# hjsuh94/irs_mpc

Hardware: AMD Instinct MI355X
Metric: rollouts*timesteps/s (randomized-smoothing pass) + iLQR-iters/s (higher is better)
Workload: dtype f32; 1 GPU; planar_hand quasi-dynamic contact, zero-order-B smoothing, step QP solved exactly (dual active-set method) -- the metric's config; T=50, N_per_gpu=10000, N_total=10000, mode=ZERO_ORDER_B, contact_solver=exact, samples=supplied, resident in HBM (f32), parallelism=samples sharded over 1 GPU(s), 1 all-reduce of (T,P) f64 per step

## Files before the change

irs_mpc_amd/csrc/reduce.hpp:

```cpp
#pragma once
#include <hip/hip_runtime.h>

constexpr int irs_reduce_pad(int P) {
    if (P > 32) return (P + 63) / 64 * 64;
    int q = 1;
    while (q < P) q <<= 1;
    return q;
}

template <int LEN, int STAGE>
struct WaveReduce {
    static constexpr bool HALVE = (LEN % 2 == 0);
    static constexpr int NEXT = HALVE ? LEN / 2 : LEN;
    static constexpr int FINAL_LEN = WaveReduce<NEXT, STAGE + 1>::FINAL_LEN;

    __device__ __forceinline__ static void run(float* v, int lane) {
        constexpr int mask = 32 >> STAGE;
        if constexpr (HALVE) {
            const bool upper = (lane & mask) != 0;
#pragma unroll
            for (int i = 0; i < LEN / 2; ++i) {
                float keep = upper ? v[i + LEN / 2] : v[i];
                float send = upper ? v[i] : v[i + LEN / 2];
                v[i] = keep + __shfl_xor(send, mask, 64);
            }
        } else {
#pragma unroll
            for (int i = 0; i < LEN; ++i) v[i] += __shfl_xor(v[i], mask, 64);
        }
        WaveReduce<NEXT, STAGE + 1>::run(v, lane);
    }
    __device__ __forceinline__ static int base(int lane) {
        constexpr int mask = 32 >> STAGE;
        int rest = WaveReduce<NEXT, STAGE + 1>::base(lane);
        if constexpr (HALVE) {
            return (rest < 0) ? -1 : rest + ((lane & mask) ? LEN / 2 : 0);
        } else {
            return (lane & mask) ? -1 : rest;
        }
    }
};
template <int LEN>
struct WaveReduce<LEN, 6> {
    static constexpr int FINAL_LEN = LEN;
    __device__ __forceinline__ static void run(float*, int) {}
    __device__ __forceinline__ static int base(int) { return 0; }
};

template <int P, int NW>
__device__ __forceinline__ void block_reduce_lds(float* acc, float* red) {
    constexpr int PP = irs_reduce_pad(P);
    using WR = WaveReduce<PP, 0>;
    const int tid = threadIdx.x;
    const int lane = tid & 63, wave = tid >> 6;
    WR::run(acc, lane);
    const int b = WR::base(lane);
    if (b >= 0) {
#pragma unroll
        for (int i = 0; i < WR::FINAL_LEN; ++i) red[wave * PP + b + i] = acc[i];
    }
}
```

irs_mpc_amd/csrc/smooth_common.hpp:

```cpp
#pragma once
#include <type_traits>
#include <cstdlib>
#include "irs_common.hpp"
#include "philox.hpp"
#include "reduce.hpp"

struct SmoothArgs {
    ModelParams p;
    const double* x_trj;
    const double* u_trj;
    const float* dx;
    const float* du;
    float std[32];
    unsigned long long seed;
    unsigned long long sample_offset;
    unsigned int iter;
    int T, N, chunk, nblk, block;
    int diag;
    int* counters;
    float* partial;
    double* fnom;
    int chunk0;
    int wg0_rr;
    double* sums;
// ... 258 lines not shown
        if (lane == 0) {
#pragma unroll
            for (int k = 0; k < n; ++k) L.fd[k] = f[k] - (double)(float)x[k];
        }
        wave_sync();
        for (int q = lane; q < NZ * n; q += 64) {
            double hq = S[TR::NG + q];
            if constexpr (TR::SUMZ) hq -= S[TR::NH + q / n] * L.fd[q % n];
            L.H[q / n][q % n] = hq;
        }
        wave_sync();
        if (lane < NZ) {
            double g = L.G[lane][lane];
            L.sc[lane] = g > 0.0 ? 1.0 / sqrt(g) : 0.0;
            if (!(g > 0.0)) L.bad = lane + 1;
        }
        wave_sync();
        for (int q = lane; q < NZ * NZ; q += 64) L.G[q / NZ][q % NZ] *= L.sc[q / NZ] * L.sc[q % NZ];
        for (int q = lane; q < NZ * n; q += 64) L.H[q / n][q % n] *= L.sc[q / n];
        wave_sync();
        static_assert(NZ <= 32 && n <= 32, "lane split of the scaling step");
        for (int j = 0; j < NZ; ++j) {
            double djj = L.G[j][j];
            if (!(djj > 1e-14)) {
                if (lane == 0 && L.bad == 0) L.bad = j + 1;
                djj = 1.0;
            }
            const double il = fast_rsqrt(djj);
            wave_sync();
            if (lane == j) L.G[j][j] = il;
            if (lane > j && lane < NZ) L.G[lane][j] *= il;
            if (lane >= 32 && lane < 32 + n) L.H[j][lane - 32] *= il;
            wave_sync();
            for (int q = lane; q < NZ * NZ; q += 64) {
                int r = q / NZ, c = q % NZ;
                if (c > j && r >= c) L.G[r][c] -= L.G[r][j] * L.G[c][j];
            }
            for (int q = lane; q < NZ * n; q += 64) {
                int r = q / n, k = q % n;
                if (r > j) L.H[r][k] -= L.G[r][j] * L.H[j][k];
            }
            wave_sync();
        }
        for (int i = NZ - 1; i >= 0; --i) {
            const double il = L.G[i][i];
            wave_sync();
            if (lane < n) L.H[i][lane] *= il;
            wave_sync();
            for (int q = lane; q < i * n; q += 64) {
                int r = q / n, k = q % n;
                L.H[r][k] -= L.G[i][r] * L.H[i][k];
            }
        }
        wave_sync();
        for (int q = lane; q < NZ * n; q += 64) L.AB[q % n][Z0 + q / n] = L.H[q / n][q % n] * L.sc[q / n];
        }
    }
    wave_sync();
    if constexpr ((MODE == IRS_SMOOTH_ZERO_ORDER_B && !Model::HAS_JACOBIAN) || TR::FIRST_B) {
        for (int q = lane; q < m * m; q += 64) L.AB[Model::u_into_x(q / m)][n + q % m] = (q / m == q % m) ? 1.0 : 0.0;
        wave_sync();
    }
    for (int q = lane; q < n * n; q += 64) At[(size_t)t * n * n + q] = L.AB[q / n][q % n];
    for (int q = lane; q < n * m; q += 64) Bt[(size_t)t * n * m + q] = L.AB[q / m][n + q % m];
    if (lane < n) {
        double c = f[0];
#pragma unroll
        for (int i = 0; i < n; ++i) c = (i == lane) ? f[i] : c;
#pragma unroll
        for (int i = 0; i < n; ++i) c -= L.AB[lane][i] * x[i];
#pragma unroll
        for (int j = 0; j < m; ++j) c -= L.AB[lane][n + j] * u[j];
        ct[(size_t)t * n + lane] = c;
    }
    {
        bool nonfinite = false;
        for (int q = lane; q < TR::P; q += 64) {
            const unsigned long long bits = (unsigned long long)__double_as_longlong(S[q]);
            nonfinite = nonfinite || ((bits & 0x7ff0000000000000ull) == 0x7ff0000000000000ull);
        }
        if (__any(nonfinite) && lane == 0) L.bad = TR::P + 1;
    }
    wave_sync();
    if (lane == 0) info[t] = L.bad;
}

struct SmoothRow {
    const ModelParams& p;
    const double* x_trj;
    const double* u_trj;
    const float* dx;
    const float* du;
    float std[32];
    unsigned long long seed, sample_offset;
    unsigned int iter;
    int T, N, chunk, nblk, block, diag;
    int* counters;
    float* partial;
    double* fnom;
    int chunk0, wg0_rr;
    double* sums;
    double* At;
    double* Bt;
    double* ct;
    int* info;
    double n_total;
    int t;
};

template <class Model, int MODE>
__device__ __forceinline__ SmoothRow smooth_batch_row(const SmoothArgs& a, const SmoothBatch& bat, int row) {
    using TR = SmoothTraits<Model, MODE>;
    constexpr int n = TR::n, m = TR::m;
    const int b = row / a.T;
    const long long wsb = b * bat.ws_stride;
    const size_t rows = (size_t)b * a.T;
    SmoothRow r{.p = a.p,
                .x_trj = a.x_trj + b * bat.x_stride,
                .u_trj = a.u_trj + b * bat.u_stride,
                .dx = nullptr, .du = nullptr,
                .std = {},
                .seed = bat.seed[b], .sample_offset = 0ull, .iter = a.iter,
                .T = a.T, .N = a.N, .chunk = a.chunk, .nblk = a.nblk, .block = a.block, .diag = a.diag,
                .counters = reinterpret_cast<int*>(reinterpret_cast<char*>(a.counters) + wsb),
                .partial = reinterpret_cast<float*>(reinterpret_cast<char*>(a.partial) + wsb),
                .fnom = reinterpret_cast<double*>(reinterpret_cast<char*>(a.fnom) + wsb),
                .chunk0 = a.chunk0, .wg0_rr = a.wg0_rr,
                .sums = a.sums + rows * TR::P, .At = a.At + rows * (n * n), .Bt = a.Bt + rows * (n * m),
                .ct = a.ct + rows * n, .info = a.info + rows,
                .n_total = a.n_total, .t = row - b * a.T};
#pragma unroll
    for (int j = 0; j < m; ++j)
        r.std[n + j] = __int_as_float(__builtin_amdgcn_readfirstlane(__float_as_int((float)bat.std_u[(size_t)b * m + j])));
    return r;
}

template <class Model, int MODE>
__device__ __forceinline__ const SmoothArgs& smooth_row(const SmoothArgs& a, const SmoothSolo&, int) { return a; }
template <class Model, int MODE>
__device__ __forceinline__ SmoothRow smooth_row(const SmoothArgs& a, const SmoothBatch& bat, int row) {
    return smooth_batch_row<Model, MODE>(a, bat, row);
}
__device__ __forceinline__ int smooth_row_t(const SmoothArgs&, int row) { return row; }
__device__ __forceinline__ int smooth_row_t(const SmoothRow& r, int) { return r.t; }

template <class Model, class = void>
struct contact_rows_of { static constexpr int value = 0; };
template <class Model>
struct contact_rows_of<Model, std::void_t<decltype(Model::NC)>> { static constexpr int value = Model::NC; };
template <class Model>
constexpr int contact_rows() { return contact_rows_of<Model>::value; }


template <class Model, int MODE, bool FUSE, int BLOCK, bool FNOM_ONLY = false, class Args = SmoothArgs>
__device__ __forceinline__ void smooth_finish(const Args& a, float* red, double* red64, double* tot,
                                              FinalizeLds<Model, MODE>& fin, int& s_ticket, int t, int blk, int tid,
                                              const double* fnom_t) {
    using TR = SmoothTraits<Model, MODE>;
    constexpr int n = TR::n, P = TR::P;
    constexpr int NW = BLOCK / 64;
    constexpr int P4 = (P + 3) / 4 * 4;
    (void)n;
    __syncthreads();

    const int nblk = a.nblk;
    if (nblk == 1) {
        for (int q = tid; q < P; q += BLOCK) {
            float s = red[q];
#pragma unroll
            for (int w = 1; w < NW; ++w) s += red[w * TR::PP + q];
            tot[q] = (double)s;
        }
    } else if constexpr (BLOCK <= 512 || FNOM_ONLY) {
        for (int q = tid; q < P; q += BLOCK) {
            float s = red[q];
#pragma unroll
            for (int w = 1; w < NW; ++w) s += red[w * TR::PP + q];
            red[q] = s;
        }
        __syncthreads();
        {
            typedef unsigned int u32x4 __attribute__((ext_vector_type(4)));
            const unsigned bytes = (unsigned)((size_t)a.T * nblk * P4 * sizeof(float));
            __amdgpu_buffer_rsrc_t rsrc = __builtin_amdgcn_make_buffer_rsrc(a.partial, 0, bytes, 0x00020000);
            const unsigned row = (unsigned)(((size_t)t * nblk + blk) * P4 * sizeof(float));
            for (int q4 = tid; q4 < P4 / 4; q4 += BLOCK) {
                u32x4 v;
                v.x = __float_as_uint(red[4 * q4]);
                v.y = __float_as_uint(red[4 * q4 + 1]);
                v.z = __float_as_uint(red[4 * q4 + 2]);
                v.w = __float_as_uint(red[4 * q4 + 3]);
                __builtin_amdgcn_raw_buffer_store_b128(v, rsrc, row + 16u * q4, 0, 16 );
            }
        }
        asm volatile("s_waitcnt vmcnt(0)" ::: "memory");
        __syncthreads();
        if (tid == 0)
            s_ticket = __hip_atomic_fetch_add(a.counters + t, 1, __ATOMIC_RELAXED, __HIP_MEMORY_SCOPE_AGENT);
        __syncthreads();
        if (s_ticket != nblk - 1) return;
        if (tid == 0) {
            __hip_atomic_store(a.counters + t, 0, __ATOMIC_RELAXED, __HIP_MEMORY_SCOPE_AGENT);
            __builtin_amdgcn_fence(__ATOMIC_ACQUIRE, "agent");
        }
        asm volatile("s_waitcnt vmcnt(0)" ::: "memory");
        __syncthreads();
        const float* src = a.partial + (size_t)t * nblk * P4;
        if constexpr (P >= kBlock) {
            for (int q = tid; q < P; q += BLOCK) {
                double s = 0.0;
#pragma unroll 8
                for (int b = 0; b < nblk; ++b) s += (double)src[(size_t)b * P4 + q];
                tot[q] = s;
            }
        } else {
            const int g = tid / P, q = tid % P;
            if (g < TR::NGRP) {
                double s = 0.0;
#pragma unroll 4
                for (int b = g; b < nblk; b += TR::NGRP) s += (double)src[(size_t)b * P4 + q];
                red64[g * P + q] = s;
            }
            __syncthreads();
            if (tid < P) {
                double s = red64[tid];
                for (int gg = 1; gg < TR::NGRP; ++gg) s += red64[gg * P + tid];
                tot[tid] = s;
            }
        }
    }
    __syncthreads();
    for (int q = tid; q < P; q += BLOCK) a.sums[(size_t)t * P + q] = tot[q];
    if constexpr (FUSE) {
        if (tid < 64 && a.diag != 1)
            finalize_timestep<Model, MODE, FNOM_ONLY>(a.p, a.x_trj, a.u_trj, tot, a.n_total, t, tid, fin, a.At, a.Bt,
                                           a.ct, a.info,
                                           fnom_t);
    }
}

}
```

irs_mpc_amd/csrc/smooth_ug.hip:

```cpp
#include "smooth_common.hpp"

namespace {

#ifndef IRS_UG_SWEEPS
#define IRS_UG_SWEEPS 6
#endif
#ifndef IRS_UG_PDAS
#define IRS_UG_PDAS 4
#endif
#ifndef IRS_UG_BLOCK
#define IRS_UG_BLOCK 512
#endif
constexpr int kUgBlock = IRS_UG_BLOCK;
constexpr int kUgSweeps = IRS_UG_SWEEPS;
constexpr int kUgPdas = IRS_UG_PDAS;
#ifndef IRS_UG_STEP_COLUMNS
#define IRS_UG_STEP_COLUMNS 1
#endif
constexpr bool kUgStepColumns = IRS_UG_STEP_COLUMNS != 0;
constexpr int kUgTabH = 8, kUgTabTau = 40, kUgTabSet = 48, kUgTabX = 52;
constexpr int kUgTabStride = 116;
#ifndef IRS_UG_NOM_ROUNDS
#define IRS_UG_NOM_ROUNDS 2
#endif
constexpr int kUgNomRounds = IRS_UG_NOM_ROUNDS;
constexpr int kUgRing = 128;

template <class Model>
struct alignas(16) UgLds {
    static constexpr int NC = Model::NC, n = Model::NX, m = Model::NU;
    float tab[1 << NC][kUgTabStride];
    float W[NC][NC];
    float invw[NC];
    float Wd[NC];
    float r0[NC];
    float phi[NC];
    float C[m][NC];
    float JD[n][NC];
    float Jc[NC][n];
    float Dinv[n];
    float Db0[n];
    float DK[m];
    float q[n];
};

__device__ __forceinline__ float ug_uniform(float v) {
    return __int_as_float(__builtin_amdgcn_readfirstlane(__float_as_int(v)));
}

template <int NC>
struct UgUni {
    float W[NC * (NC + 1) / 2];
    float invw[NC];
    float r0[NC];
    __device__ __forceinline__ float w(int i, int j) const {
        return i <= j ? W[i * NC - i * (i - 1) / 2 + (j - i)] : W[j * NC - j * (j - 1) / 2 + (i - j)];
    }
};

template <class Model>
__device__ __forceinline__ unsigned ug_lookup_affine(const UgLds<Model>& S, unsigned a, const float* du, float tol,
                                                     float* v, float* tau) {
    constexpr int NC = Model::NC, m = Model::NU;
    static_assert(NC == 8 && m == 4, "table entries are 8 rows by 4 commands");
    const float4* e = reinterpret_cast<const float4*>(&S.tab[a][0]);
    float4 g4[kUgTabSet / 4];
#pragma unroll
    for (int c = 0; c < kUgTabSet / 4; ++c) g4[c] = e[c];
    const unsigned ap = __float_as_uint(S.tab[a][kUgTabSet]);
    tau[0] = g4[kUgTabTau / 4].x; tau[1] = g4[kUgTabTau / 4].y; tau[2] = g4[kUgTabTau / 4].z; tau[3] = g4[kUgTabTau / 4].w;
    tau[4] = g4[kUgTabTau / 4 + 1].x; tau[5] = g4[kUgTabTau / 4 + 1].y; tau[6] = g4[kUgTabTau / 4 + 1].z; tau[7] = g4[kUgTabTau / 4 + 1].w;
    v[0] = fmaf(tau[0], tol, g4[0].x); v[1] = fmaf(tau[1], tol, g4[0].y);
    v[2] = fmaf(tau[2], tol, g4[0].z); v[3] = fmaf(tau[3], tol, g4[0].w);
    v[4] = fmaf(tau[4], tol, g4[1].x); v[5] = fmaf(tau[5], tol, g4[1].y);
    v[6] = fmaf(tau[6], tol, g4[1].z); v[7] = fmaf(tau[7], tol, g4[1].w);
#pragma unroll
    for (int j = 0; j < m; ++j) {
        const float4 lo = g4[kUgTabH / 4 + 2 * j], hi = g4[kUgTabH / 4 + 2 * j + 1];
        v[0] = fmaf(lo.x, du[j], v[0]); v[1] = fmaf(lo.y, du[j], v[1]);
        v[2] = fmaf(lo.z, du[j], v[2]); v[3] = fmaf(lo.w, du[j], v[3]);
        v[4] = fmaf(hi.x, du[j], v[4]); v[5] = fmaf(hi.y, du[j], v[5]);
        v[6] = fmaf(hi.z, du[j], v[6]); v[7] = fmaf(hi.w, du[j], v[7]);
    }
    return ap;
}

template <class Model, bool UCOL>
__device__ __forceinline__ void ug_step_direction(const UgLds<Model>& S, unsigned a, int p, float* u, float* tau) {
    constexpr int NC = Model::NC;
    const float* e = &S.tab[a][0];
    const float4 t0 = *reinterpret_cast<const float4*>(e + kUgTabTau), t1 = *reinterpret_cast<const float4*>(e + kUgTabTau + 4);
    if constexpr (UCOL) {
        const float4 lo = *reinterpret_cast<const float4*>(e + kUgTabX + NC * p);
        const float4 hi = *reinterpret_cast<const float4*>(e + kUgTabX + NC * p + 4);
        u[0] = lo.x; u[1] = lo.y; u[2] = lo.z; u[3] = lo.w;
        u[4] = hi.x; u[5] = hi.y; u[6] = hi.z; u[7] = hi.w;
    } else {
        const float4 wlo = *reinterpret_cast<const float4*>(&S.W[p][0]);
        const float4 whi = *reinterpret_cast<const float4*>(&S.W[p][4]);
        const float4* x4 = reinterpret_cast<const float4*>(e + kUgTabX);
        float4 g4[2 * NC];
#pragma unroll
        for (int c = 0; c < 2 * NC; ++c) g4[c] = x4[c];
        const float wp[NC] = {wlo.x, wlo.y, wlo.z, wlo.w, whi.x, whi.y, whi.z, whi.w};
#pragma unroll
        for (int i = 0; i < NC; ++i) u[i] = 0.f;
#pragma unroll
        for (int c = 0; c < NC; ++c) {
            const float4 lo = g4[2 * c], hi = g4[2 * c + 1];
            u[0] = fmaf(lo.x, wp[c], u[0]); u[1] = fmaf(lo.y, wp[c], u[1]);
            u[2] = fmaf(lo.z, wp[c], u[2]); u[3] = fmaf(lo.w, wp[c], u[3]);
            u[4] = fmaf(hi.x, wp[c], u[4]); u[5] = fmaf(hi.y, wp[c], u[5]);
            u[6] = fmaf(hi.z, wp[c], u[6]); u[7] = fmaf(hi.w, wp[c], u[7]);
        }
    }
    tau[0] = t0.x; tau[1] = t0.y; tau[2] = t0.z; tau[3] = t0.w;
    tau[4] = t1.x; tau[5] = t1.y; tau[6] = t1.z; tau[7] = t1.w;
}

template <class Model>
__device__ __forceinline__ float ug_rhs(const UgUni<Model::NC>& U, const UgLds<Model>& S, const float* du, float* r) {
    constexpr int NC = Model::NC, m = Model::NU;
#pragma unroll
    for (int c = 0; c < NC; ++c) r[c] = U.r0[c];
#pragma unroll
    for (int j = 0; j < m; ++j) {
        const float4 lo = *reinterpret_cast<const float4*>(&S.C[j][0]);
        const float4 hi = *reinterpret_cast<const float4*>(&S.C[j][4]);
        r[0] = fmaf(lo.x, du[j], r[0]); r[1] = fmaf(lo.y, du[j], r[1]);
        r[2] = fmaf(lo.z, du[j], r[2]); r[3] = fmaf(lo.w, du[j], r[3]);
        r[4] = fmaf(hi.x, du[j], r[4]); r[5] = fmaf(hi.y, du[j], r[5]);
        r[6] = fmaf(hi.z, du[j], r[6]); r[7] = fmaf(hi.w, du[j], r[7]);
    }
    float scale = 1e-30f;
#pragma unroll
    for (int c = 0; c < NC; ++c) scale = fmaxf(scale, fabsf(r[c]));
    return 1e-6f * scale;
}

template <class Model>
__device__ __forceinline__ bool ug_try(const UgUni<Model::NC>& U, const UgLds<Model>& S, const float* r, const float* du,
                                       float tolv, float* lam, unsigned& a_out, int diag = 0) {
    constexpr int NC = Model::NC;
    float g[NC];
#pragma unroll
    for (int i = 0; i < NC; ++i) { lam[i] = 0.f; g[i] = r[i]; }
#pragma unroll 2
    for (int sw = 0; sw < ((diag & 64) ? 0 : kUgSweeps); ++sw) {
#pragma unroll
        for (int i = 0; i < NC; ++i) {
            const float nw = fmaxf(fmaf(-g[i], U.invw[i], lam[i]), 0.f);
            const float dl = nw - lam[i];
            lam[i] = nw;
#pragma unroll
            for (int j = 0; j < NC; ++j) g[j] = fmaf(U.w(j, i), dl, g[j]);
        }
    }
    unsigned a = 0u;
#pragma unroll
    for (int i = 0; i < NC; ++i) a |= (lam[i] > 0.f) ? (1u << i) : 0u;
    bool done = (diag & 32) != 0;
    for (int it = 0; it < kUgPdas; ++it) {
        float v[NC], tau[NC];
        const unsigned ap = ug_lookup_affine<Model>(S, a, du, tolv, v, tau);
        unsigned bad = 0u;
#pragma unroll
        for (int i = NC - 1; i >= 0; --i) bad = __builtin_amdgcn_alignbit(bad, __float_as_uint(v[i]), 31);
        if (!done) {
            if (bad == 0u) {
#pragma unroll
                for (int i = 0; i < NC; ++i) lam[i] = fmaf(-tau[i], v[i], v[i]);
                done = true;
            }
            a = ap ^ bad;
        }
        if (__all(done)) break;
    }
    a_out = a;
    return done;
}

template <class Model, bool UCOL>
__device__ __forceinline__ void ug_full(const UgLds<Model>& S, const float* r, const float* du, float tolv, unsigned a,
                                        float* lam, int cap = 4 * Model::NC) {
    constexpr int NC = Model::NC;
    constexpr float kBig = 3.0e38f, piv_rel = 1e-5f;
    float g[NC];
    bool valid = false;
    for (int round = 0; round < 3; ++round) {
        if (__all(valid)) break;
        float v[NC], tau[NC];
        const unsigned ap = ug_lookup_affine<Model>(S, a, du, 0.f, v, tau);
        if (!valid) {
            unsigned negb = 0u;
#pragma unroll
            for (int i = 0; i < NC; ++i) {
                const bool in = tau[i] == 0.f;
                negb |= (in && !(v[i] > 0.f)) ? (1u << i) : 0u;
                lam[i] = in ? v[i] : 0.f;
                g[i] = in ? 0.f : v[i];
            }
            valid = negb == 0u;
            a = ap & ~negb;
        }
    }
    if (!valid) {
        a = 0u;
#pragma unroll
        for (int i = 0; i < NC; ++i) { lam[i] = 0.f; g[i] = r[i]; }
    }
    int p = -1;
    bool done = false;
    for (int it = 0; it < cap; ++it) {
        if (!done && p < 0) {
            float vmin = kBig;
            int c = 0;
#pragma unroll
            for (int i = 0; i < NC; ++i) {
                const float vv = ((a >> i) & 1u) ? kBig : g[i];
                if (vv < vmin) { vmin = vv; c = i; }
            }
            if (vmin >= -tolv) done = true;
            else p = c;
        }
        if (__all(done)) break;
        const int pp = (done || p < 0) ? 0 : p;
        float u[NC], tau[NC];
        ug_step_direction<Model, UCOL>(S, a, pp, u, tau);
        const float wpp = S.Wd[pp];
        float gp = 0.f, zp = 0.f;
#pragma unroll
        for (int i = 0; i < NC; ++i) {
            const bool isp = i == pp;
            gp = isp ? g[i] : gp;
            zp = isp ? u[i] : zp;
        }
        const bool full_ok = zp > piv_rel * wpp;
        const float t2 = full_ok ? -gp * irs_rcp_fast(zp) : kBig;
        float rho[NC], qv[NC];
        float t1 = kBig;
#pragma unroll
        for (int i = 0; i < NC; ++i) {
            rho[i] = fmaf(tau[i], u[i], -u[i]);
            qv[i] = rho[i] > 0.f ? lam[i] * irs_rcp_fast(rho[i]) : kBig;
            t1 = fminf(t1, qv[i]);
        }
        int kb = 0;
#pragma unroll
        for (int i = NC - 1; i >= 0; --i) kb = (qv[i] == t1) ? i : kb;
        const float tmin = fminf(t1, t2);
        if (!done && !(tmin < kBig)) done = true;
        const float tt = done ? 0.f : tmin;
#pragma unroll
        for (int i = 0; i < NC; ++i) {
            g[i] = fmaf(tt * tau[i], u[i], g[i]);
            lam[i] = fmaxf(fmaf(-tt, rho[i], lam[i]) + ((i == pp) ? tt : 0.f), 0.f);
        }
        if (!done) {
            const bool full = t2 <= t1;
            if (full) {
                a |= 1u << pp;
                p = -1;
            } else {
                a &= ~(1u << kb);
#pragma unroll
                for (int i = 0; i < NC; ++i) lam[i] = (i == kb) ? 0.f : lam[i];
            }
        }
    }
}

template <class Model, bool UCOL>
__device__ __forceinline__ void ug_build_entry(UgLds<Model>& S, unsigned a, int half) {
    constexpr int NC = Model::NC;
    constexpr float piv_rel = 1e-5f;
    float M_[NC][NC], inv[NC], W[NC][NC];
    bool act[NC];
#pragma unroll
    for (int i = 0; i < NC; ++i) {
        act[i] = ((a >> i) & 1u) != 0u;
#pragma unroll
        for (int j = 0; j < NC; ++j) W[i][j] = S.W[i][j];
#pragma unroll
        for (int j = 0; j <= i; ++j) M_[i][j] = W[i][j];
    }
    unsigned ap = 0u;
#pragma unroll
    for (int j = 0; j < NC; ++j) {
        const float dj = M_[j][j];
        const bool ok = act[j] && dj > piv_rel * W[j][j];
        act[j] = ok;
        ap |= ok ? (1u << j) : 0u;
        inv[j] = ok ? irs_rcp_fast(dj) : 0.f;
#pragma unroll
        for (int i = j + 1; i < NC; ++i) M_[j][i] = M_[i][j] * inv[j];
#pragma unroll
        for (int i = j + 1; i < NC; ++i)
#pragma unroll
            for (int k = j + 1; k <= i; ++k) M_[i][k] = M_[i][k] - M_[j][i] * M_[k][j];
    }
    float* e = &S.tab[a][0];
    constexpr int NAPP = 1 + Model::NU + NC, SHARE = (NAPP + 1) / 2;
    for (int qq = 0; qq < SHARE; ++qq) {
        const int q = half * SHARE + qq;
        if (q >= NAPP) break;
        const int c = q - (1 + Model::NU);
        float x[NC];
        if (UCOL || c < 0) {
            const float* src = q == 0 ? &S.r0[0] : (c < 0 ? &S.C[q - 1][0] : &S.W[c][0]);
            const float4 lo = *reinterpret_cast<const float4*>(src), hi = *reinterpret_cast<const float4*>(src + 4);
            x[0] = lo.x; x[1] = lo.y; x[2] = lo.z; x[3] = lo.w;
            x[4] = hi.x; x[5] = hi.y; x[6] = hi.z; x[7] = hi.w;
        } else {
#pragma unroll
            for (int i = 0; i < NC; ++i) x[i] = (i == c) ? 1.f : 0.f;
        }
        float y[NC];
#pragma unroll
        for (int j = 0; j < NC; ++j) {
            float v = act[j] ? -x[j] : 0.f;
#pragma unroll
            for (int k = 0; k < j; ++k) v = v - M_[k][j] * y[k];
            y[j] = v;
        }
#pragma unroll
        for (int j = NC - 1; j >= 0; --j) {
            float v = y[j] * inv[j];
#pragma unroll
            for (int i = j + 1; i < NC; ++i) v = v - M_[j][i] * y[i];
            y[j] = v;
        }
        float col[NC];
#pragma unroll
        for (int i = 0; i < NC; ++i) {
            float s = x[i];
#pragma unroll
            for (int j = 0; j < NC; ++j) s = fmaf(W[i][j], y[j], s);
            col[i] = act[i] ? y[i] : s;
        }
        float* dst = e + (c < 0 ? NC * q : kUgTabX + NC * c);
        *reinterpret_cast<float4*>(dst) = make_float4(col[0], col[1], col[2], col[3]);
        *reinterpret_cast<float4*>(dst + 4) = make_float4(col[4], col[5], col[6], col[7]);
    }
    if (half == 1) {
        *reinterpret_cast<float4*>(e + kUgTabTau) = make_float4(act[0] ? 0.f : 1.f, act[1] ? 0.f : 1.f, act[2] ? 0.f : 1.f, act[3] ? 0.f : 1.f);
        *reinterpret_cast<float4*>(e + kUgTabTau + 4) = make_float4(act[4] ? 0.f : 1.f, act[5] ? 0.f : 1.f, act[6] ? 0.f : 1.f, act[7] ? 0.f : 1.f);
        e[kUgTabSet] = __uint_as_float(ap);
    }
}

struct UgNomLds {
    double J[8][7];
    double q[7], Dinv[7], b[7];
};

template <class Model, class Args>
__device__ __forceinline__ double ug_nominal_geometry(const Args& a, UgNomLds& L, int t, int lane) {
    constexpr int NC = Model::NC, n = Model::NX, m = Model::NU;
    double x64[n], u64[m], q[n], Dinv[n], b[n], J[NC][n], phi[NC];
#pragma unroll
    for (int i = 0; i < n; ++i) x64[i] = a.x_trj[(size_t)t * n + i];
#pragma unroll
    for (int j = 0; j < m; ++j) u64[j] = a.u_trj[(size_t)t * m + j];
    Model::template assemble<double>(a.p, x64, u64, q, Dinv, b, J, phi);
    if (lane == 0) {
#pragma unroll
        for (int c = 0; c < NC; ++c)
#pragma unroll
            for (int k = 0; k < n; ++k) L.J[c][k] = J[c][k];
#pragma unroll
        for (int k = 0; k < n; ++k) { L.q[k] = q[k]; L.Dinv[k] = Dinv[k]; L.b[k] = b[k]; }
    }
    double rr = 0.0;
#pragma unroll
    for (int c = 0; c < NC; ++c) {
        double s = phi[c];
#pragma unroll
        for (int k = 0; k < n; ++k) s -= J[c][k] * (b[k] * Dinv[k]);
        rr = (lane == c) ? s : rr;
    }
    wave_sync();
    return rr;
}

template <class Model, bool UCOL, class Args>
__device__ __forceinline__ void ug_nominal(const Args& a, const UgUni<Model::NC>& U, const UgLds<Model>& S,
                                           UgNomLds& L, double rr, int t, int lane) {
    constexpr int NC = Model::NC, n = Model::NX, m = Model::NU;
    static_assert(NC == 8 && n <= 8, "lane (i,k) = 8 i + k owns entry (i,k) of the 8 x 8 dual Hessian");
    float du0[m], r32[NC], lam32[NC];
#pragma unroll
    for (int j = 0; j < m; ++j) du0[j] = 0.f;
    const float tolv = ug_rhs<Model>(U, S, du0, r32);
    unsigned am = 0u;
    if (!ug_try<Model>(U, S, r32, du0, tolv, lam32, am)) ug_full<Model, UCOL>(S, r32, du0, tolv, am, lam32);
    unsigned set = 0u;
#pragma unroll
    for (int i = 0; i < NC; ++i) set |= (lam32[i] > 0.f) ? (1u << i) : 0u;
    set = (unsigned)__builtin_amdgcn_readfirstlane((int)set);
    {
        const int li = lane >> 3, lk = lane & 7;
        double w = 0.0;
#pragma unroll
        for (int kk = 0; kk < n; ++kk) w += L.J[li][kk] * L.Dinv[kk] * L.J[lk][kk];
        double scale = 1e-300;
#pragma unroll
        for (int c = 0; c < NC; ++c) scale = fmax(scale, fabs(__shfl(rr, c, 64)));
        const double tol64 = 1e-10 * scale;
        double lamd = 0.0;
        bool settled = false;
        for (int corr = 0; corr < 8 && !settled; ++corr) {
            double M = w, Lf = 0.0;
            unsigned eff = 0u;
            double invd[NC];
#pragma unroll
            for (int j = 0; j < NC; ++j) {
                const double dj = __shfl(M, 9 * j, 64), wjj = __shfl(w, 9 * j, 64);
                const bool ok = ((set >> j) & 1u) && dj > 1e-7 * wjj;
                eff |= ok ? (1u << j) : 0u;
                invd[j] = ok ? 1.0 / dj : 0.0;
                const double Mij = __shfl(M, 8 * li + j, 64), Mkj = __shfl(M, 8 * lk + j, 64);
                if (lk == j && li > j) Lf = Mij * invd[j];
                if (li > j && lk > j) M -= Mij * invd[j] * Mkj;
            }
            const bool mine = lane < NC && ((eff >> lane) & 1u);
            double y = mine ? -rr : 0.0;
#pragma unroll
            for (int j = 0; j < NC; ++j) {
                const double yj = __shfl(y, j, 64);
                const double Lij = __shfl(Lf, 8 * (lane & 7) + j, 64);
                if (lane < NC && lane > j) y -= Lij * yj;
            }
            double invme = 0.0;
#pragma unroll
            for (int j = 0; j < NC; ++j) invme = (lane == j) ? invd[j] : invme;
            y *= invme;
#pragma unroll
            for (int j = NC - 1; j >= 0; --j) {
                const double yj = __shfl(y, j, 64);
                const double Lji = __shfl(Lf, 8 * j + (lane & 7), 64);
                if (lane < j) y -= Lji * yj;
            }
            lamd = mine ? y : 0.0;
            double pr = w * __shfl(lamd, lk, 64);
            pr += __shfl_xor(pr, 1, 64);
            pr += __shfl_xor(pr, 2, 64);
            pr += __shfl_xor(pr, 4, 64);
            const double sl = rr + __shfl(pr, 8 * (lane & 7), 64);
            const bool neg = lane < NC && mine && !(lamd > 0.0);
            const bool viol = lane < NC && !mine && sl < -tol64;
            const unsigned negb = (unsigned)(__ballot(neg) & 0xffull), violb = (unsigned)(__ballot(viol) & 0xffull);
            if ((negb | violb) == 0u) settled = true;
            else set = (eff & ~negb) | violb;
        }
        double f = 0.0;
        if (settled) {
            double acc = 0.0;
#pragma unroll
            for (int c = 0; c < NC; ++c) acc += L.J[c][lane < n ? lane : 0] * __shfl(lamd, c, 64);
            if (lane < n) f = L.q[lane] + L.Dinv[lane] * (acc - L.b[lane]);
        } else if (lane < n) {
            float acc = -S.Db0[lane];
#pragma unroll
            for (int c = 0; c < NC; ++c) acc = fmaf(S.JD[lane][c], lam32[c], acc);
            f = (double)(S.q[lane] + acc);
        }
        if (lane < n)
            __hip_atomic_store(a.fnom + (size_t)t * n + Model::perm(lane), f, __ATOMIC_RELAXED, __HIP_MEMORY_SCOPE_AGENT);
    }
}

#ifdef IRS_UG_STAMPS
constexpr int kUgStampSlots = 12, kUgStampWgs = 2048;
__device__ unsigned long long ug_stamps[kUgStampWgs * kUgStampSlots];
#define UG_STAMP(slot)                                                                          \
    do {                                                                                        \
        if ((threadIdx.x & 63) == 0) {                                                          \
            const int wg_ = blockIdx.y * gridDim.x + blockIdx.x;                                \
            if (wg_ < kUgStampWgs && ((slot) < 8 ? threadIdx.x == 0 : true))                    \
                ug_stamps[wg_ * kUgStampSlots + (slot)] = __builtin_amdgcn_s_memtime();         \
        }                                                                                       \
    } while (0)
#else
#define UG_STAMP(slot) do {} while (0)
#endif

template <class Model, int MODE, bool RNG, bool FUSE, bool BATCH>
__global__ __launch_bounds__(kUgBlock) void smooth_ug_kernel(SmoothArgs args, std::conditional_t<BATCH, SmoothBatch, SmoothSolo> bat) {
    using TR = SmoothTraits<Model, MODE>;
    constexpr int n = TR::n, m = TR::m, P = TR::P, NC = Model::NC;
    constexpr int BLOCK = kUgBlock, NW = BLOCK / 64;
    static_assert(TR::Z0 == n && NC == 8 && m == 4, "u-only smoothing of an 8-row contact model with 4 commands");
    static_assert(P < kBlock, "the hand-off's group reduction");
    constexpr int NG = m * (m + 1) / 2;
    constexpr int PI = TR::FIRST_B ? 1 : NG + m * NC + m;
    constexpr int PPI = irs_reduce_pad(TR::FIRST_B ? n * m : PI);
    constexpr int QE = m + 1;
    constexpr bool UCOL = !TR::FIRST_B && kUgStepColumns;
    __shared__ UgLds<Model> S;
    __shared__ UgNomLds nomL;
    __shared__ float ring_all[NW * kUgRing * QE];
    __shared__ float red[NW * (PPI > TR::PP ? PPI : TR::PP)];
    __shared__ float toti[PPI];
    __shared__ unsigned hist[TR::FIRST_B ? (1 << NC) : 1];
    __shared__ double red64[TR::NGRP * P];
    __shared__ double tot[P];
    __shared__ FinalizeLds<Model, MODE> fin;
    __shared__ int s_ticket;

    decltype(auto) a = smooth_row<Model, MODE>(args, bat, (int)blockIdx.y);
    const int t = smooth_row_t(a, (int)blockIdx.y), blk = blockIdx.x, tid = threadIdx.x;
    const int lane = tid & 63, wave = tid >> 6;

    UG_STAMP(0);
    const bool nominal_wave = blk == 0 && wave == NW - 1;
    double nom_r = 0.0;
    if (nominal_wave && !(a.diag & 2)) nom_r = ug_nominal_geometry<Model>(a, nomL, t, lane);
    if (wave == 0) {
        float xb[n], ub[m], q[n], Dinv[n], b0[n], J[NC][n], phi[NC];
#pragma unroll
        for (int i = 0; i < n; ++i) xb[i] = (float)a.x_trj[(size_t)t * n + i];
#pragma unroll
        for (int j = 0; j < m; ++j) ub[j] = (float)a.u_trj[(size_t)t * m + j];
        Model::template assemble<float>(a.p, xb, ub, q, Dinv, b0, J, phi);
        if (lane == 0) {
#pragma unroll
            for (int i = 0; i < NC; ++i) {
                S.phi[i] = phi[i];
#pragma unroll
                for (int k = 0; k < n; ++k) S.Jc[i][k] = J[i][k];
            }
#pragma unroll
            for (int k = 0; k < n; ++k) { S.Db0[k] = b0[k] * Dinv[k]; S.q[k] = q[k]; S.Dinv[k] = Dinv[k]; }
#pragma unroll
            for (int j = 0; j < m; ++j) S.DK[j] = Dinv[Model::act(j)] * Model::template stiffness<float>(a.p, j);
        }
    }
    if constexpr (TR::FIRST_B) {
        for (int q = tid; q < (1 << NC); q += BLOCK) hist[q] = 0u;
    }
    __syncthreads();
    if (tid < NC * NC) {
        const int i = tid / NC, j = tid % NC, hi = i > j ? i : j, lo = i > j ? j : i;
        float w = (S.Jc[hi][0] * S.Dinv[0]) * S.Jc[lo][0];
#pragma unroll
        for (int k = 1; k < n; ++k) w = w + (S.Jc[hi][k] * S.Dinv[k]) * S.Jc[lo][k];
        S.W[i][j] = w;
        if (i == j) {
            S.Wd[i] = w;
            S.invw[i] = (float)kContactPgsOmega * irs_rcp_fast(w);
        }
    } else if (tid < NC * NC + NC) {
        const int i = tid - NC * NC;
        float ri = S.phi[i];
#pragma unroll
        for (int k = 0; k < n; ++k) ri = ri - S.Jc[i][k] * S.Db0[k];
        S.r0[i] = ri;
    } else if (tid < 2 * NC * NC + NC) {
        const int e = tid - (NC * NC + NC), k = e / NC, c = e % NC;
        if (k < n) S.JD[k][c] = S.Jc[c][k] * S.Dinv[k];
    } else if (tid < 2 * NC * NC + NC + m * NC) {
        const int e = tid - (2 * NC * NC + NC), j = e / NC, c = e % NC;
        S.C[j][c] = (S.Jc[c][Model::act(j)] * S.Dinv[Model::act(j)]) * Model::template stiffness<float>(a.p, j);
    }
    __syncthreads();
    UG_STAMP(1);
    if (!(a.diag & 4))
        for (int e = tid; e < 2 * (1 << NC); e += BLOCK) ug_build_entry<Model, UCOL>(S, (unsigned)(e >> 1), e & 1);
    __syncthreads();

    UG_STAMP(2);
    UgUni<NC> U;
    {
        int q = 0;
#pragma unroll
        for (int i = 0; i < NC; ++i)
#pragma unroll
            for (int j = i; j < NC; ++j) U.W[q++] = S.W[i][j];
#pragma unroll
        for (int i = 0; i < NC; ++i) { U.invw[i] = S.invw[i]; U.r0[i] = S.r0[i]; }
    }

    float acc[PPI];
#pragma unroll
    for (int i = 0; i < PPI; ++i) acc[i] = 0.f;

    if (nominal_wave && !(a.diag & 2)) ug_nominal<Model, UCOL>(a, U, S, nomL, nom_r, t, lane);
    if (nominal_wave) UG_STAMP(8);
    if (!(a.diag & 8)) {
        const int V = a.nblk * NW;
        const int me = nominal_wave ? V - 1 : (blk == 0 ? wave : blk * NW - 1 + wave);
        const int nblocks = (a.N + 63) / 64;
        int round = nominal_wave ? kUgNomRounds : 0;
        auto block_of = [&](int k) { return k < kUgNomRounds ? k * (V - 1) + me : kUgNomRounds * (V - 1) + (k - kUgNomRounds) * V + me; };
        float* ring = ring_all + wave * (kUgRing * QE);
        int qhead = 0, qtail = 0;
        int bk = block_of(round);
        float du_next[m];
#pragma unroll
        for (int j = 0; j < m; ++j) du_next[j] = 0.f;
        auto request = [&](int block) {
            if constexpr (!RNG) {
                if (block < nblocks) {
                    const int sidx = block * 64 + lane;
                    const size_t row = (size_t)t * a.N + (sidx < a.N ? sidx : a.N - 1);
                    load_row<m>(a.du + row * m, du_next);
                }
            }
        };
        request(bk);
        while (true) {
            const bool fresh = bk < nblocks;
            const int pending = qtail - qhead;
            const bool flush = pending >= 64 || (!fresh && pending > 0);
            if (!fresh && !flush) break;
            float du[m], r[NC], lam[NC];
            bool on, fin_ = true;
            if (flush) {
                __builtin_amdgcn_fence(__ATOMIC_RELEASE, "wavefront");
                __builtin_amdgcn_wave_barrier();
                __builtin_amdgcn_fence(__ATOMIC_ACQUIRE, "wavefront");
                const int take = min(64, pending);
                on = lane < take;
                const int slot = (qhead + (on ? lane : 0)) & (kUgRing - 1);
#pragma unroll
                for (int j = 0; j < m; ++j) du[j] = ring[slot * QE + j];
                const unsigned wm = __float_as_uint(ring[slot * QE + m]);
                const float tolv = ug_rhs<Model>(U, S, du, r);
                ug_full<Model, UCOL>(S, r, du, tolv, wm, lam, (a.diag & 128) ? 8 : ((a.diag & 256) ? 12 : 4 * NC));
                qhead += take;
            } else {
                const int sidx = bk * 64 + lane;
                on = sidx < a.N;
                if constexpr (RNG) {
                    const unsigned long long gidx = a.sample_offset + (unsigned long long)sidx;
#pragma unroll
                    for (int j = n / 4; j < (n + m + 3) / 4; ++j) {
                        float g4[4];
                        philox_normal4(gidx, (unsigned)t, (unsigned)j, a.iter, a.seed, g4);
#pragma unroll
                        for (int c = 0; c < 4; ++c) {
                            const int idx = 4 * j + c;
                            if (idx >= n && idx < n + m) du[idx - n] = __fmul_rn(g4[c], a.std[idx]);
                        }
                    }
                } else {
#pragma unroll
                    for (int j = 0; j < m; ++j) du[j] = du_next[j];
                    request(block_of(round + 1));
                }
                const float tolv = ug_rhs<Model>(U, S, du, r);
                unsigned mask = 0u;
                fin_ = ug_try<Model>(U, S, r, du, tolv, lam, mask, a.diag);
                if (a.diag & 16) fin_ = true;
                const bool hard = on && !fin_;
                const unsigned long long bal = __ballot(hard);
                if (hard) {
                    const int slot = (qtail + __popcll(bal & ((1ull << lane) - 1ull))) & (kUgRing - 1);
#pragma unroll
                    for (int j = 0; j < m; ++j) ring[slot * QE + j] = du[j];
                    ring[slot * QE + m] = __uint_as_float(mask);
                }
                qtail += __popcll(bal);
                bk = block_of(++round);
            }
            const bool use = on && fin_;
            bool nonfinite = false;
#pragma unroll
            for (int j = 0; j < m; ++j) nonfinite = nonfinite || irs_nonfinite_bits(du[j]);
            if constexpr (TR::FIRST_B) {
                unsigned I = 0u;
#pragma unroll
                for (int i = 0; i < NC; ++i) I |= (lam[i] * S.Wd[i] > (float)kContactActiveTol) ? (1u << i) : 0u;
                if (use) __hip_atomic_fetch_add(&hist[I], 1u, __ATOMIC_RELAXED, __HIP_MEMORY_SCOPE_WORKGROUP);
                if (on && nonfinite) acc[0] = irs_poison();
            } else {
                float zz[m];
#pragma unroll
                for (int j = 0; j < m; ++j) zz[j] = use ? du[j] : 0.f;
                int q = 0;
#pragma unroll
                for (int i = 0; i < m; ++i)
#pragma unroll
                    for (int j = i; j < m; ++j) { acc[q] = fmaf(zz[i], zz[j], acc[q]); ++q; }
#pragma unroll
                for (int i = 0; i < m; ++i)
#pragma unroll
                    for (int c = 0; c < NC; ++c) { acc[q] = fmaf(zz[i], lam[c], acc[q]); ++q; }
#pragma unroll
                for (int i = 0; i < m; ++i) { acc[q] += zz[i]; ++q; }
                if (on && nonfinite) acc[0] = irs_poison();
            }
        }
    }

    UG_STAMP(3);
    if (blk == 0 && wave == 1) UG_STAMP(9);
    if constexpr (TR::FIRST_B) {
        __syncthreads();
        unsigned poison_bits = __float_as_uint(acc[0]);
        asm volatile("" : "+v"(poison_bits));
#pragma unroll
        for (int i = 0; i < PPI; ++i) acc[i] = 0.f;
        for (int I = tid; I < (1 << NC); I += BLOCK) {
            const unsigned cnt = hist[I];
            if (cnt == 0u) continue;
            const float* e = &S.tab[I][0];
            const unsigned ap = __float_as_uint(e[kUgTabSet]);
            float Y[NC][m];
#pragma unroll
            for (int i = 0; i < NC; ++i) {
                const bool in = ((ap >> i) & 1u) != 0u;
#pragma unroll
                for (int c = 0; c < m; ++c) {
                    float s = 0.f;
#pragma unroll
                    for (int j = 0; j < NC; ++j) s = fmaf(e[kUgTabX + 8 * j + i], S.Jc[j][Model::act(c)], s);
                    Y[i][c] = in ? -s : 0.f;
                }
            }
#pragma unroll
            for (int k = 0; k < n; ++k)
#pragma unroll
                for (int c = 0; c < m; ++c) {
                    float s = 0.f;
#pragma unroll
                    for (int i = 0; i < NC; ++i) s = fmaf(S.Jc[i][k], Y[i][c], s);
                    const float Bkc = (k == Model::act(c) ? 1.f : 0.f) - S.Dinv[k] * s;
                    acc[Model::perm(k) * m + c] += (float)cnt * Bkc;
                }
        }
        if ((poison_bits & 0x7f800000u) == 0x7f800000u) acc[0] = irs_poison();
        block_reduce_lds<P, NW>(acc, red);
    } else {
        block_reduce_lds<PI, NW>(acc, red);
        __syncthreads();
        for (int q = tid; q < PI; q += BLOCK) {
            float s = red[q];
#pragma unroll
            for (int w = 1; w < NW; ++w) s += red[w * PPI + q];
            toti[q] = s;
        }
        __syncthreads();
        float out = 0.f;
        if (tid < P) {
            if (tid < NG) out = toti[tid];
            else if (tid < NG + m * n) {
                const int i = (tid - NG) / n, kext = (tid - NG) % n;
                int k = 0, jact = -1;
#pragma unroll
                for (int kk = 0; kk < n; ++kk) k = (Model::perm(kk) == kext) ? kk : k;
#pragma unroll
                for (int j = 0; j < m; ++j) jact = (Model::act(j) == k) ? j : jact;
                float s = -S.Db0[k] * toti[NG + m * NC + i];
                for (int c = 0; c < NC; ++c) s = fmaf(S.JD[k][c], toti[NG + i * NC + c], s);
                if (jact >= 0) {
                    const int lo = i < jact ? i : jact, hi = i < jact ? jact : i;
                    s = fmaf(S.DK[jact], toti[lo * m - lo * (lo - 1) / 2 + (hi - lo)], s);
                }
                out = s;
            } else {
                out = toti[NG + m * NC + (tid - NG - m * n)];
            }
        }
        __syncthreads();
        for (int q = tid; q < NW * TR::PP; q += BLOCK) red[q] = 0.f;
        __syncthreads();
        if (tid < P) red[tid] = out;
    }
    UG_STAMP(4);
    smooth_finish<Model, MODE, FUSE, BLOCK, true, std::remove_cv_t<std::remove_reference_t<decltype(a)>>>(a, red, red64, tot, fin, s_ticket, t, blk, tid, a.fnom + (size_t)t * n);
    UG_STAMP(5);
}

template <class Model, int MODE>
void ug_launch_m(const SmoothArgs& a, bool rng, bool fuse, hipStream_t st) {
    dim3 grid(a.nblk, a.T), block(kUgBlock);
    if (rng) {
        if (fuse) hipLaunchKernelGGL((smooth_ug_kernel<Model, MODE, true, true, false>), grid, block, 0, st, a, SmoothSolo{});
        else hipLaunchKernelGGL((smooth_ug_kernel<Model, MODE, true, false, false>), grid, block, 0, st, a, SmoothSolo{});
    } else {
        if (fuse) hipLaunchKernelGGL((smooth_ug_kernel<Model, MODE, false, true, false>), grid, block, 0, st, a, SmoothSolo{});
        else hipLaunchKernelGGL((smooth_ug_kernel<Model, MODE, false, false, false>), grid, block, 0, st, a, SmoothSolo{});
    }
}

template <class Model, int MODE>
void ug_launch_batch_m(const SmoothArgs& a, const SmoothBatch& bat, int B, hipStream_t st) {
    dim3 grid(a.nblk, B * a.T), block(kUgBlock);
    hipLaunchKernelGGL((smooth_ug_kernel<Model, MODE, true, true, true>), grid, block, 0, st, a, bat);
}

}

#ifdef IRS_UG_STAMPS
extern "C" int irs_debug_ug_stamps(unsigned long long* host_out, int n_wgs) {
    if (n_wgs > kUgStampWgs) n_wgs = kUgStampWgs;
    return (int)hipMemcpyFromSymbol(host_out, HIP_SYMBOL(ug_stamps), (size_t)n_wgs * kUgStampSlots * sizeof(unsigned long long));
}
#endif

bool irs_smooth_ug_supported(int model, int mode) {
    const char* e = getenv("IRS_UG");
    if (e != nullptr && atoi(e) == 0) return false;
    return model == IRS_MODEL_PLANAR_HAND_EXACT && (mode == IRS_SMOOTH_ZERO_ORDER_B || mode == IRS_SMOOTH_FIRST_ORDER);
}

int irs_smooth_ug_nblk(int T, int N) {
    static int cus = 0;
    if (cus == 0) {
        hipDeviceProp_t prop;
        int dev = 0;
        cus = (hipGetDevice(&dev) == hipSuccess && hipGetDeviceProperties(&prop, dev) == hipSuccess)
                  ? prop.multiProcessorCount : 256;
        if (cus < 1) cus = 256;
    }
    const int nblocks = (N + 63) / 64, NW = kUgBlock / 64;
    int nb = cus / (T < 1 ? 1 : T);
    if (nb < 1) nb = 1;
    const int by_work = (nblocks + 1 + NW - 1) / NW;
    if (nb > by_work) nb = by_work;
    return nb < 1 ? 1 : nb;
}

int irs_smooth_ug_launch(int model, int mode, const SmoothArgs& a, bool rng, bool fuse, hipStream_t st) {
    if (model != IRS_MODEL_PLANAR_HAND_EXACT) return IRS_ERR_UNSUPPORTED;
    if (mode == IRS_SMOOTH_ZERO_ORDER_B) ug_launch_m<PlanarHandExactModel, IRS_SMOOTH_ZERO_ORDER_B>(a, rng, fuse, st);
    else if (mode == IRS_SMOOTH_FIRST_ORDER) ug_launch_m<PlanarHandExactModel, IRS_SMOOTH_FIRST_ORDER>(a, rng, fuse, st);
    else return IRS_ERR_UNSUPPORTED;
    return IRS_OK;
}

int irs_smooth_ug_launch_batch(int model, int mode, const SmoothArgs& a, const SmoothBatch& bat, int B, hipStream_t st) {
    if (model != IRS_MODEL_PLANAR_HAND_EXACT) return IRS_ERR_UNSUPPORTED;
    if (mode == IRS_SMOOTH_ZERO_ORDER_B) ug_launch_batch_m<PlanarHandExactModel, IRS_SMOOTH_ZERO_ORDER_B>(a, bat, B, st);
    else if (mode == IRS_SMOOTH_FIRST_ORDER) ug_launch_batch_m<PlanarHandExactModel, IRS_SMOOTH_FIRST_ORDER>(a, bat, B, st);
    else return IRS_ERR_UNSUPPORTED;
    return IRS_OK;
}
```

Before: 13.89 billion rollouts*timesteps/s.

## Build only live table columns, peel last sweep, trim reduction padding and syncs

Table entries are now assigned to lanes in popcount-ranked order, and each entry builds only the columns its active set needs, writing identity columns for the rest, so the warps stay balanced. The last projected Gauss-Seidel sweep is peeled so it updates only the remaining gradients. The reduction uses a tighter pad of 16 and the row-0 finish skips the re-summation of the per-wave partials and two barriers. The risks are correctness: the skipped table columns and the missing zeroing must never be read, and the new static_assert fixes the block at 512 with 8 contacts.

Measured after the change: 14.35 billion rollouts*timesteps/s (median of 5 runs). +3.4%, better.

```diff
diff --git a/irs_mpc_amd/csrc/reduce.hpp b/irs_mpc_amd/csrc/reduce.hpp
--- a/irs_mpc_amd/csrc/reduce.hpp
+++ b/irs_mpc_amd/csrc/reduce.hpp
@@ -47,9 +47,9 @@
     __device__ __forceinline__ static int base(int) { return 0; }
 };
 
-template <int P, int NW>
+template <int P, int NW, int PP = irs_reduce_pad(P)>
 __device__ __forceinline__ void block_reduce_lds(float* acc, float* red) {
-    constexpr int PP = irs_reduce_pad(P);
+    static_assert(PP >= P, "the padding holds every accumulator");
     using WR = WaveReduce<PP, 0>;
     const int tid = threadIdx.x;
     const int lane = tid & 63, wave = tid >> 6;
diff --git a/irs_mpc_amd/csrc/smooth_common.hpp b/irs_mpc_amd/csrc/smooth_common.hpp
--- a/irs_mpc_amd/csrc/smooth_common.hpp
+++ b/irs_mpc_amd/csrc/smooth_common.hpp
@@ -434,7 +434,7 @@
 constexpr int contact_rows() { return contact_rows_of<Model>::value; }
 
 
-template <class Model, int MODE, bool FUSE, int BLOCK, bool FNOM_ONLY = false, class Args = SmoothArgs>
+template <class Model, int MODE, bool FUSE, int BLOCK, bool FNOM_ONLY = false, class Args = SmoothArgs, bool ROW0 = false>
 __device__ __forceinline__ void smooth_finish(const Args& a, float* red, double* red64, double* tot,
                                               FinalizeLds<Model, MODE>& fin, int& s_ticket, int t, int blk, int tid,
                                               const double* fnom_t) {
@@ -449,18 +449,22 @@
     if (nblk == 1) {
         for (int q = tid; q < P; q += BLOCK) {
             float s = red[q];
-#pragma unroll
-            for (int w = 1; w < NW; ++w) s += red[w * TR::PP + q];
+            if constexpr (!ROW0) {
+#pragma unroll
+                for (int w = 1; w < NW; ++w) s += red[w * TR::PP + q];
+            }
             tot[q] = (double)s;
         }
     } else if constexpr (BLOCK <= 512 || FNOM_ONLY) {
-        for (int q = tid; q < P; q += BLOCK) {
-            float s = red[q];
-#pragma unroll
-            for (int w = 1; w < NW; ++w) s += red[w * TR::PP + q];
-            red[q] = s;
-        }
-        __syncthreads();
+        if constexpr (!ROW0) {
+            for (int q = tid; q < P; q += BLOCK) {
+                float s = red[q];
+#pragma unroll
+                for (int w = 1; w < NW; ++w) s += red[w * TR::PP + q];
+                red[q] = s;
+            }
+            __syncthreads();
+        }
         {
             typedef unsigned int u32x4 __attribute__((ext_vector_type(4)));
             const unsigned bytes = (unsigned)((size_t)a.T * nblk * P4 * sizeof(float));
diff --git a/irs_mpc_amd/csrc/smooth_ug.hip b/irs_mpc_amd/csrc/smooth_ug.hip
--- a/irs_mpc_amd/csrc/smooth_ug.hip
+++ b/irs_mpc_amd/csrc/smooth_ug.hip
@@ -86,13 +86,14 @@
 }
 
 template <class Model, bool UCOL>
-__device__ __forceinline__ void ug_step_direction(const UgLds<Model>& S, unsigned a, int p, float* u, float* tau) {
+__device__ __forceinline__ void ug_step_direction(const UgLds<Model>& S, unsigned a, int p, bool idle, float* u, float* tau) {
     constexpr int NC = Model::NC;
     const float* e = &S.tab[a][0];
     const float4 t0 = *reinterpret_cast<const float4*>(e + kUgTabTau), t1 = *reinterpret_cast<const float4*>(e + kUgTabTau + 4);
     if constexpr (UCOL) {
-        const float4 lo = *reinterpret_cast<const float4*>(e + kUgTabX + NC * p);
-        const float4 hi = *reinterpret_cast<const float4*>(e + kUgTabX + NC * p + 4);
+        const int off = idle ? 0 : kUgTabX + NC * p;
+        const float4 lo = *reinterpret_cast<const float4*>(e + off);
+        const float4 hi = *reinterpret_cast<const float4*>(e + off + 4);
         u[0] = lo.x; u[1] = lo.y; u[2] = lo.z; u[3] = lo.w;
         u[4] = hi.x; u[5] = hi.y; u[6] = hi.z; u[7] = hi.w;
     } else {
@@ -145,8 +146,9 @@
     float g[NC];
 #pragma unroll
     for (int i = 0; i < NC; ++i) { lam[i] = 0.f; g[i] = r[i]; }
+    const int nsw = (diag & 64) ? 0 : kUgSweeps;
 #pragma unroll 2
-    for (int sw = 0; sw < ((diag & 64) ? 0 : kUgSweeps); ++sw) {
+    for (int sw = 0; sw < nsw - 1; ++sw) {
 #pragma unroll
         for (int i = 0; i < NC; ++i) {
             const float nw = fmaxf(fmaf(-g[i], U.invw[i], lam[i]), 0.f);
@@ -154,6 +156,16 @@
             lam[i] = nw;
 #pragma unroll
             for (int j = 0; j < NC; ++j) g[j] = fmaf(U.w(j, i), dl, g[j]);
+        }
+    }
+    if (nsw > 0) {
+#pragma unroll
+        for (int i = 0; i < NC; ++i) {
+            const float nw = fmaxf(fmaf(-g[i], U.invw[i], lam[i]), 0.f);
+            const float dl = nw - lam[i];
+            lam[i] = nw;
+#pragma unroll
+            for (int j = i + 1; j < NC; ++j) g[j] = fmaf(U.w(j, i), dl, g[j]);
         }
     }
     unsigned a = 0u;
@@ -224,9 +236,10 @@
             else p = c;
         }
         if (__all(done)) break;
-        const int pp = (done || p < 0) ? 0 : p;
+        const bool idle = done || p < 0;
+        const int pp = idle ? 0 : p;
         float u[NC], tau[NC];
-        ug_step_direction<Model, UCOL>(S, a, pp, u, tau);
+        ug_step_direction<Model, UCOL>(S, a, pp, idle, u, tau);
         const float wpp = S.Wd[pp];
         float gp = 0.f, zp = 0.f;
 #pragma unroll
@@ -270,8 +283,22 @@
     }
 }
 
+struct UgRank { unsigned char entry[256]; };
+constexpr UgRank ug_rank_by_popcount() {
+    UgRank r{};
+    int q = 0;
+    for (int pc = 0; pc <= 8; ++pc)
+        for (int a = 0; a < 256; ++a) {
+            int c = 0;
+            for (int i = 0; i < 8; ++i) c += (a >> i) & 1;
+            if (c == pc) r.entry[q++] = (unsigned char)a;
+        }
+    return r;
+}
+__device__ constexpr UgRank kUgRank = ug_rank_by_popcount();
+
 template <class Model, bool UCOL>
-__device__ __forceinline__ void ug_build_entry(UgLds<Model>& S, unsigned a, int half) {
+__device__ __forceinline__ void ug_build_entry(UgLds<Model>& S, unsigned a, int half, bool full) {
     constexpr int NC = Model::NC;
     constexpr float piv_rel = 1e-5f;
     float M_[NC][NC], inv[NC], W[NC][NC];
@@ -300,11 +327,19 @@
             for (int k = j + 1; k <= i; ++k) M_[i][k] = M_[i][k] - M_[j][i] * M_[k][j];
     }
     float* e = &S.tab[a][0];
-    constexpr int NAPP = 1 + Model::NU + NC, SHARE = (NAPP + 1) / 2;
-    for (int qq = 0; qq < SHARE; ++qq) {
-        const int q = half * SHARE + qq;
-        if (q >= NAPP) break;
-        const int c = q - (1 + Model::NU);
+    constexpr int NFIX = 1 + Model::NU;
+    const unsigned live = full ? 0xffu : (UCOL ? ~a & 0xffu : a);
+    const int L = NFIX + __popc(live);
+    unsigned rest = half == 0 ? live & (live - 1u) : live;
+    for (int it = half; __any(it < L); it += 2) {
+        if (it >= L) continue;
+        int q = it;
+        if (it >= NFIX) {
+            q = NFIX + __ffs(rest) - 1;
+            rest &= rest - 1u;
+            rest &= rest - 1u;
+        }
+        const int c = q - NFIX;
         float x[NC];
         if (UCOL || c < 0) {
             const float* src = q == 0 ? &S.r0[0] : (c < 0 ? &S.C[q - 1][0] : &S.W[c][0]);
@@ -341,6 +376,14 @@
         float* dst = e + (c < 0 ? NC * q : kUgTabX + NC * c);
         *reinterpret_cast<float4*>(dst) = make_float4(col[0], col[1], col[2], col[3]);
         *reinterpret_cast<float4*>(dst + 4) = make_float4(col[4], col[5], col[6], col[7]);
+    }
+    if constexpr (!UCOL) {
+#pragma unroll
+        for (int j = 0; j < NC; ++j)
+            if (!((live >> j) & 1u) && (j & 1) == half) {
+                *reinterpret_cast<float4*>(e + kUgTabX + NC * j) = make_float4(j == 0 ? 1.f : 0.f, j == 1 ? 1.f : 0.f, j == 2 ? 1.f : 0.f, j == 3 ? 1.f : 0.f);
+                *reinterpret_cast<float4*>(e + kUgTabX + NC * j + 4) = make_float4(j == 4 ? 1.f : 0.f, j == 5 ? 1.f : 0.f, j == 6 ? 1.f : 0.f, j == 7 ? 1.f : 0.f);
+            }
     }
     if (half == 1) {
         *reinterpret_cast<float4*>(e + kUgTabTau) = make_float4(act[0] ? 0.f : 1.f, act[1] ? 0.f : 1.f, act[2] ? 0.f : 1.f, act[3] ? 0.f : 1.f);
@@ -477,7 +520,7 @@
     do {                                                                                        \
         if ((threadIdx.x & 63) == 0) {                                                          \
             const int wg_ = blockIdx.y * gridDim.x + blockIdx.x;                                \
-            if (wg_ < kUgStampWgs && ((slot) < 8 ? threadIdx.x == 0 : true))                    \
+            if (wg_ < kUgStampWgs && (((slot) < 8 || (slot) == 10) ? threadIdx.x == 0 : true))  \
                 ug_stamps[wg_ * kUgStampSlots + (slot)] = __builtin_amdgcn_s_memtime();         \
         }                                                                                       \
     } while (0)
@@ -494,7 +537,7 @@
     static_assert(P < kBlock, "the hand-off's group reduction");
     constexpr int NG = m * (m + 1) / 2;
     constexpr int PI = TR::FIRST_B ? 1 : NG + m * NC + m;
-    constexpr int PPI = irs_reduce_pad(TR::FIRST_B ? n * m : PI);
+    constexpr int PPI = TR::FIRST_B ? irs_reduce_pad(n * m) : (PI + 15) / 16 * 16;
     constexpr int QE = m + 1;
     constexpr bool UCOL = !TR::FIRST_B && kUgStepColumns;
     __shared__ UgLds<Model> S;
@@ -510,10 +553,12 @@
 
     decltype(auto) a = smooth_row<Model, MODE>(args, bat, (int)blockIdx.y);
     const int t = smooth_row_t(a, (int)blockIdx.y), blk = blockIdx.x, tid = threadIdx.x;
-    const int lane = tid & 63, wave = tid >> 6;
+    const int lane = tid & 63, wave = __builtin_amdgcn_readfirstlane(tid >> 6);
 
     UG_STAMP(0);
     const bool nominal_wave = blk == 0 && wave == NW - 1;
+    static_assert(BLOCK == 512 && NC == 8, "two lanes per table entry, 32 entries per wave");
+    const unsigned tab_entry = kUgRank.entry[(wave < 4 ? wave : 11 - wave) * 32 + (lane >> 1)];
     double nom_r = 0.0;
     if (nominal_wave && !(a.diag & 2)) nom_r = ug_nominal_geometry<Model>(a, nomL, t, lane);
     if (wave == 0) {
@@ -565,8 +610,7 @@
     }
     __syncthreads();
     UG_STAMP(1);
-    if (!(a.diag & 4))
-        for (int e = tid; e < 2 * (1 << NC); e += BLOCK) ug_build_entry<Model, UCOL>(S, (unsigned)(e >> 1), e & 1);
+    if (!(a.diag & 4)) ug_build_entry<Model, UCOL>(S, tab_entry, lane & 1, (a.diag & 512) != 0);
     __syncthreads();
 
     UG_STAMP(2);
@@ -698,6 +742,7 @@
     if (blk == 0 && wave == 1) UG_STAMP(9);
     if constexpr (TR::FIRST_B) {
         __syncthreads();
+        UG_STAMP(10);
         unsigned poison_bits = __float_as_uint(acc[0]);
         asm volatile("" : "+v"(poison_bits));
 #pragma unroll
@@ -733,8 +778,9 @@
         if ((poison_bits & 0x7f800000u) == 0x7f800000u) acc[0] = irs_poison();
         block_reduce_lds<P, NW>(acc, red);
     } else {
-        block_reduce_lds<PI, NW>(acc, red);
+        block_reduce_lds<PI, NW, PPI>(acc, red);
         __syncthreads();
+        UG_STAMP(10);
         for (int q = tid; q < PI; q += BLOCK) {
             float s = red[q];
 #pragma unroll
@@ -753,6 +799,7 @@
 #pragma unroll
                 for (int j = 0; j < m; ++j) jact = (Model::act(j) == k) ? j : jact;
                 float s = -S.Db0[k] * toti[NG + m * NC + i];
+#pragma unroll
                 for (int c = 0; c < NC; ++c) s = fmaf(S.JD[k][c], toti[NG + i * NC + c], s);
                 if (jact >= 0) {
                     const int lo = i < jact ? i : jact, hi = i < jact ? jact : i;
@@ -763,13 +810,10 @@
                 out = toti[NG + m * NC + (tid - NG - m * n)];
             }
         }
-        __syncthreads();
-        for (int q = tid; q < NW * TR::PP; q += BLOCK) red[q] = 0.f;
-        __syncthreads();
-        if (tid < P) red[tid] = out;
+        if (tid < (P + 3) / 4 * 4) red[tid] = out;
     }
     UG_STAMP(4);
-    smooth_finish<Model, MODE, FUSE, BLOCK, true, std::remove_cv_t<std::remove_reference_t<decltype(a)>>>(a, red, red64, tot, fin, s_ticket, t, blk, tid, a.fnom + (size_t)t * n);
+    smooth_finish<Model, MODE, FUSE, BLOCK, true, std::remove_cv_t<std::remove_reference_t<decltype(a)>>, !TR::FIRST_B>(a, red, red64, tot, fin, s_ticket, t, blk, tid, a.fnom + (size_t)t * n);
     UG_STAMP(5);
 }
 
```
